# iglu-contest/gridworld

Measured on AMD Instinct MI355X. Metric: env-steps/sec (render=False, vector_state) at N parallel envs, 1/2/4/8 GPU, higher is better.
Workload: dtype f64

## Files before the change

__graft_entry__.py:

```python
import os
import sys

ROOT = os.path.dirname(os.path.abspath(__file__))
if ROOT not in sys.path:
    sys.path.insert(0, ROOT)


def build():
    from gridworld_amd import build as hip_build, codec as hip_codec, goal as hip_goal, query as hip_query, render as hip_render
    lib = hip_build.build(force=True)
    assert os.path.exists(lib)
    assert os.path.exists(hip_render.build(force=True))
    assert os.path.exists(hip_codec.build(force=True))
    assert os.path.exists(hip_query.build(force=True))
    assert os.path.exists(hip_goal.build(force=True))
    from oracle import oracle as O
    O.build(force=True)
    import gridworld_amd
    from gridworld_amd import _lib
    L = _lib.load()
    assert L.igw_version() == _lib.VERSION
    print('built', lib, 'and', O._LIB_PATH)


def smoke():
    import numpy as np
    import torch
    from gridworld_amd import VecGridWorld, workloads
    from oracle import oracle as O
    assert torch.cuda.is_available(), 'smoke() needs a GPU'

    def same(env, ob, n):
        torch.cuda.synchronize()
        assert np.array_equal(env.grid.cpu().numpy().reshape(n, -1), ob.grid)
        assert np.array_equal(env.agent_pos.cpu().numpy().view(np.uint32), ob.agentPos.view(np.uint32))
        assert np.array_equal(env.reward.cpu().numpy(), ob.reward) and np.array_equal(env.done.cpu().numpy(), ob.done)
        assert np.array_equal(env.inventory.cpu().numpy(), ob.inventory)
        assert np.array_equal(env.internals().view(np.uint64), ob.internals().view(np.uint64))

    n, T = 64, 60
    tg = workloads.rt20(n, seed=3).numpy()
    kw = dict(size_reward=False, max_steps=40)
    env = VecGridWorld(n, device='cuda:0', autoreset=True, **kw)
    env.set_tasks(tg)
# ... 42 lines not shown
```

gridworld_amd/_lib.py:

```python
import ctypes as C
import os

HERE = os.path.dirname(os.path.abspath(__file__))
LIB_PATH = os.path.join(HERE, 'libigw_hip.so')

GRID_STRIDE = 1104
CELLS = 1089
AGENT_BYTES = 64
AUX_BYTES = 16
OUT_BYTES = 64
TASK_META_BYTES = 128
OCC_WORDS = 48
TRAJ_BYTES = 64
HIST_ROW = 512
STAT_STRIPES = 64
STAT_CHANGED, STAT_RESETS, STAT_STEPS, STAT_RESCANS, STAT_BAD_POSE, STAT_BAD_ACTION, STAT_BAD_TASK = 0, 1, 2, 3, 4, 5, 6
VERSION = 5
LEVEL_INDEX_BYTES = 160
TASK_INDEX_BYTES = 9 * LEVEL_INDEX_BYTES
WALKING_DISCRETE, FLYING, WALKING_DICT = 0, 1, 2
RESET_KEEP_SIZE = 1
CAMERA_MAX = 1e6
AUTO_32_MAX, AUTO_16_MAX, AUTO_8_MAX = 1024, 4096, 24576

# ... 20 lines not shown


class Buffers(C.Structure):
    _fields_ = [(n, C.c_void_p) for n in ('grid', 'occ', 'hist', 'agent', 'aux', 'task_target', 'task_start',
                                          'task_start_occ', 'task_meta', 'task_index', 'out', 'stats')]


_lib = None


def load(build_if_missing=True):
    global _lib
    if _lib is not None:
        return _lib
    diag = os.environ.get('IGW_DIAG') == '1'
    path = os.path.join(HERE, 'libigw_hip_diag.so') if diag else LIB_PATH
    if os.environ.get('IGW_LIB'):
        path, build_if_missing = os.environ['IGW_LIB'], False
    if build_if_missing:
        from . import build as _build
        (_build.DIAG if diag else _build.STEP).build_for_load(IgwError)
    if not os.path.exists(path):
        raise IgwError(f'{os.path.basename(path)} not found; run `python -m gridworld_amd.build`')
    L = C.CDLL(path)
    vp, i32, i64, u64 = C.c_void_p, C.c_int32, C.c_int64, C.c_uint64
    L.igw_version.restype = C.c_int
    L.igw_last_error.restype = C.c_char_p
    L.igw_build_id.restype = C.c_char_p
    L.igw_device_count.restype = C.c_int
    L.igw_create.argtypes = [C.POINTER(Config), C.POINTER(vp)]
    L.igw_destroy.argtypes = [vp]
    L.igw_debug_set_stamps.argtypes = [vp, vp]
    L.igw_bind_buffers.argtypes = [vp, C.POINTER(Buffers)]
    L.igw_prepare_tasks.argtypes = [vp, i32, i32, vp, vp, vp, vp, vp, vp]
    L.igw_reset.argtypes = [vp, vp, i32, vp]
    L.igw_set_task_sampling.argtypes = [vp, i32, u64, i32]
    L.igw_set_random_tasks.argtypes = [vp, i32, u64, i32, i32, i32, i32, vp]
    L.igw_set_trajectory_log.argtypes = [vp, vp, vp, i32, i32]
    L.igw_step_walking.argtypes = [vp, vp, vp]
    L.igw_step_flying.argtypes = [vp, vp, vp, vp, vp, vp]
    L.igw_step_walking_dict.argtypes = [vp, vp, vp, vp]
    L.igw_rollout_walking.argtypes = [vp, i64, u64, i64, i64, vp]
    L.igw_rollout_walking_actions.argtypes = [vp, vp, i64, vp, vp, vp]
    L.igw_rollout_flying_actions.argtypes = [vp, vp, vp, vp, vp, i64, vp, vp, vp]
    L.igw_fill_actions_walking.argtypes = [vp, vp, i64, i64, u64, i64, vp]
    L.igw_task_eval.argtypes = [i32, i32, vp, vp, vp, vp, vp, vp, vp, vp]
    L.igw_debug_trig.argtypes = [i32, i64, vp, vp, vp, vp, vp, vp, vp]
    for name in EXPORTS:
        getattr(L, name)
        if name not in ('igw_last_error', 'igw_build_id'):
            getattr(L, name).restype = C.c_int
    _lib = L
    return L


def build_id():
    return load().igw_build_id().decode()


def check(code, what=''):
    if code != 0:
        msg = load().igw_last_error()
        raise IgwError(f'{what} failed ({code}): {msg.decode() if msg else ""}')
```

gridworld_amd/env.py:

```python
import ctypes as C
import warnings

import numpy as np
import torch

from . import _lib as L
from . import spaces
from .tasks import Task, Tasks
from .vec_env import VecGridWorld

_NO_TASK = ('Task is not initialized! Initialize task before working with the environment using .set_task '
            'method OR set tasks distribution using .set_task_generator method')
_TIS = (2, 4, 8, 12)


class AgentView:
    PAD = 0.25
    __slots__ = ('_env',)

    def __init__(self, env):
        self._env = env

    def _f64(self):
        return self._env._host['agent'][:48].view(np.float64)
# ... 137 lines not shown
            self._step_call = lambda: v.lib.igw_step_flying(v.ctx, p + 16, p + 8, p + 28, p + 32, self._stream_handle)
        elif v.walk_dict:
            self._step_call = lambda: v.lib.igw_step_walking_dict(v.ctx, p, p + 8, self._stream_handle)
        else:
            self._step_call = lambda: v.lib.igw_step_walking(v.ctx, p, self._stream_handle)
        self._read_back()
        self._frame = None
        if self.renderer_kind == 'hip':
            W, H = int(self.render_size[0]), int(self.render_size[1])
            self._frame = torch.zeros((1, H, W, 4), dtype=torch.uint8).pin_memory()

    def _launch_frame(self):
        from . import render as R
        v = self._vec
        R.render_into(v.agent_buf.data_ptr(), v.grid_buf.data_ptr(), v.occ_buf.data_ptr(), 1, v._atlas(),
                      self._frame.data_ptr(), self._frame.shape[2], self._frame.shape[1], 4, self._stream_handle)

    def _renders(self):
        return self.do_render and not self.fake and self._frame is not None

    def _device_step(self):
        rc = self._step_call()
        if rc:
            L.check(rc, 'igw_step (facade)')
        if self._renders():
            self._launch_frame()
        self._stream.synchronize()

    def _read_back(self):
        torch.cuda.current_stream(self._vec.device).synchronize()

    @property
    def unwrapped(self):
        return self

    @property
    def step_no(self):
        return int(self._host['agent'][60:62].view(np.uint16)[0])

    @property
    def grid(self):
        return self._host['grid'].reshape(9, 11, 11).astype(np.int32)

    def set_task(self, task):
        if self._task_generator is not None:
            warnings.warn('The .set_task method has no effect with an initialized tasks generator. '
                          'Drop it using .set_tasks_generator(None) after calling .set_task')
# ... 246 lines not shown
```

gridworld_amd/vec_env.py:

```python
import ctypes as C
import weakref

import numpy as np
import torch

from . import _lib as L
from . import codec as K
from . import goal as G
from . import query as Q
from . import render as R


def _as_rows(x, device, n=None):
    if x is None:
        return None
    t = torch.as_tensor(np.asarray(x) if not torch.is_tensor(x) else x)
    if t.dim() == 3:
        t = t.unsqueeze(0)
    t = t.reshape(t.shape[0], -1)
    if t.shape[1] == L.GRID_STRIDE:
        return t.to(device=device, dtype=torch.int8).contiguous()
    if t.shape[1] != L.CELLS:
        raise ValueError(f'grid rows must have 1089 cells, got {t.shape[1]}')
    out = torch.zeros((t.shape[0], L.GRID_STRIDE), dtype=torch.int8, device=device)
    out[:, :L.CELLS] = t.to(device=device, dtype=torch.int8)
    return out


def _invariant(x, n, device):
# ... 54 lines not shown
            self.dev = torch.zeros((2, self.n), dtype=torch.uint8, device=self.device)
            self.dev[0].fill_(int(root not in self.drawn))

    def captured(self, sl, restart):
        first, mask = self.dev[0, sl], self.dev[1, sl]
        if restart is None:
            mask.copy_(first)
        else:
            torch.bitwise_or(restart, first, out=mask)
        first.zero_()
        return mask


class _Rows:
    parent, lo, stream = None, 0, None

    def _root(self):
        return self if self.parent is None else self.parent

    def _open(self, cfg, stats_buf):
        root, sl = self._root(), slice(self.lo, self.lo + cfg.num_envs)
        self.cfg, self.num_envs, self.env_index_base, self.stats_buf = cfg, cfg.num_envs, cfg.env_index_base, stats_buf
        self.ctx = C.c_void_p()
        L.check(self.lib.igw_create(C.byref(cfg), C.byref(self.ctx)), 'igw_create')
        bound = [getattr(root, k)[sl] for k in _ROW_BUFFERS] + [getattr(root, k) for k in _TASK_BUFFERS] + \
            [root.out_buf[sl], stats_buf]
        L.check(self.lib.igw_bind_buffers(self.ctx, C.byref(L.Buffers(*[t.data_ptr() for t in bound]))),
                'igw_bind_buffers')
        self._sl = sl
        self._rows = (root.agent_buf[sl], root.grid_buf[sl], root.occ_buf[sl])

    def _follow_with(self, pov, mask, goal=None):
        self._pov, self._mask, self._goal = pov, mask, goal
        self.pov = pov.tensors.get('rgb') if pov else None
        self.pov_obs = pov.obs if pov else None
        self._obs = {'agentPos': self.agent_pos, 'inventory': self.inventory, 'compass': self.compass.unsqueeze(1),
                     'grid': self.grid}
        if pov is not None:
            pov.add_to(self._obs)
        if mask is not None:
            self._obs['action_mask'] = mask
        if goal is not None:
            self._obs.update(goal)
            if 'gain' in goal:
                self._goal_scratch()

    def __del__(self):
        ctx = getattr(self, 'ctx', None)
        if ctx:
            self.lib.igw_destroy(ctx)
            self.ctx = None

    def _stream(self):
        if self.stream is None:
            return C.c_void_p(torch._C._cuda_getCurrentRawStream(self._dev_index))
        return C.c_void_p(self.stream.cuda_stream)

    def _in_use(self, *tensors):
        if self.stream is not None:
            for t in tensors:
                if torch.is_tensor(t):
                    t.record_stream(self.stream)

    def _atlas(self):
        root = self._root()
        if root._render_atlas is None:
            root.set_render_atlas(None)
        return root._render_atlas

# ... 39 lines not shown
                                        torch.zeros((n, L.AGENT_BYTES), dtype=torch.uint8, device=dev),
                                        torch.zeros((n, Q.ACTIONS), dtype=torch.uint8, device=dev))
        return tmp

    def _ended(self):
        return self.done if self.autoreset else None

    def _draw(self, stream=None, restart=None, fill=False):
        pov = self._pov
        if stream is None:
            stream = self._stream()
            self._in_use(*pov.tensors.values(), pov.obs)
        if pov.obs is not None:
            _render_obs_rows(self, pov.spec, pov.obs, pov.tensors.get('rgb'), restart, fill, stream)
        elif pov.plain:
            _render_rows(self, pov.tensors['rgb'], 3, None, None, stream)
        else:
            _render_rows(self, pov.tensors, 3, None, tuple(pov.tensors), stream)

    def step_walking_ptr(self, actions_i32):
        if actions_i32.numel() != self.num_envs:
            raise _SPACES[L.WALKING_DISCRETE].mismatch('step_walking_ptr', self.num_envs, None, actions_i32)
        self._in_use(actions_i32)
        L.check(self.lib.igw_step_walking(self.ctx, actions_i32.data_ptr(), self._stream()), 'igw_step_walking')
        if self.parent is None:
            self._follow_mask()
            self._follow_goal()
        else:
            self._follow(self._ended())

    def action_mask(self, out=None, look=False, sample=None):
        self._in_use(*(out if isinstance(out, (tuple, list)) else (out,)))
        res = _mask_rows(self, out, look, sample, self._stream(), self.stream)
        self._in_use(*(res if isinstance(res, tuple) else (res,)))
        return res

    def goal(self, want=False, todo=True, gain=False, out=None):
        names = ('align', 'fit') + (('want',) if want else ()) + (('todo',) if todo else ()) + \
            (('gain', 'ends') if gain else ())
        self._in_use(*(out or {}).values())
        res = _goal_rows(self, names, out, self._stream(), self.stream)
        self._in_use(*res.values())
        return res

    def render_pov(self, out=None, channels=3, size=None, outputs=None, codec=None, quality=90):
        self._in_use(*(out.values() if isinstance(out, dict) else out if isinstance(out, (tuple, list)) else (out,)))

# ... 16 lines not shown
                 renderer=None, pov_outputs=('rgb',), pov_obs=None, pov_frame=True, action_mask=False, goal=False):
        if renderer not in (None, 'hip'):
            raise ValueError(f"unknown renderer {renderer!r}; the one renderer is 'hip'")
        pov_outputs = R.check_outputs(pov_outputs)
        if renderer is None and pov_outputs != ('rgb',):
            raise ValueError("pov_outputs needs renderer='hip'")
        if pov_obs is not None:
            if renderer is None:
                raise ValueError("pov_obs needs renderer='hip'")
            if pov_outputs != ('rgb',):
                raise ValueError("pov_obs goes with pov_outputs=('rgb',) only: the planes are not written in this layout")
            pov_obs = R.ObsSpec.of(pov_obs)
        elif not pov_frame:
            raise ValueError('pov_frame=False needs pov_obs (there would be nothing to draw)')
        if render and not fake and renderer is None:
            raise NotImplementedError("render=True needs renderer='hip' (the batched HIP ray caster of the "
                                      "first-person frame); or pass render=False")
        if not torch.cuda.is_available():
            raise L.IgwError('VecGridWorld needs a HIP device (no CPU fallback)')
        if action_space not in ('walking', 'flying'):
            raise ValueError(f'unknown action_space {action_space!r}')
        if action_mask and (action_space != 'walking' or not discretize):
            raise ValueError('action_mask=True needs the Discrete(18) walking action space')
        self.lib = L.load()
        self.device = torch.device(device)
        self.num_envs = int(num_envs)
        self.num_tasks = int(num_tasks or num_envs)
        self.flying = action_space == 'flying'
        self.walk_dict = action_space == 'walking' and not discretize
        mode = L.FLYING if self.flying else L.WALKING_DICT if self.walk_dict else L.WALKING_DISCRETE
        self._space = _SPACES[mode]
        self.max_steps = int(max_steps)
        self.autoreset = bool(autoreset)
        self.select_and_place = bool(select_and_place)
        N, T, dev = self.num_envs, self.num_tasks, self.device
        z = lambda shape, dt: torch.zeros(shape, dtype=dt, device=dev)
        rec = L.OUT_BYTES + L.AGENT_BYTES + L.AUX_BYTES
        self.host_records = bool(host_records)
        if self.host_records:
            self.host_view = torch.zeros((N * (rec + L.GRID_STRIDE),), dtype=torch.uint8).pin_memory()
        else:
            self.host_view = z((N * (rec + L.GRID_STRIDE),), torch.uint8)
        cut = lambda lo, width: self.host_view[N * lo:N * (lo + width)].view(N, width)
        self.out_buf = cut(0, L.OUT_BYTES)
        self.agent_buf = cut(L.OUT_BYTES, L.AGENT_BYTES)
        self.aux_buf = cut(L.OUT_BYTES + L.AGENT_BYTES, L.AUX_BYTES)
        self.grid_buf = cut(rec, L.GRID_STRIDE).view(torch.int8)
# ... 64 lines not shown
        dev = self.device
        tgt = _as_rows(targets, dev)
        T = tgt.shape[0]
        st = _as_rows(starts, dev)
        fg = _as_rows(full_grids, dev)
        inv = _invariant(invariant, T, dev)
        for name, g, hi in (('targets', tgt, 7), ('starts', st, 6), ('full_grids', fg, 7)):
            if g is not None and g.numel() and (int(g.min()) < 0 or int(g.max()) > hi):
                raise ValueError(f'{name}: block ids must be in 0..{hi}')
        if first < 0 or first + T > self.num_tasks:
            raise ValueError(f'task rows [{first}, {first + T}) do not fit the table of {self.num_tasks}')
        for name, g in (('starts', st), ('full_grids', fg)):
            if g is not None and g.shape[0] != T:
                raise ValueError(f'{name} has {g.shape[0]} rows, targets {T}')
        pose = None
        if init_pose is not None:
            pose_np = np.asarray(init_pose, dtype=np.float64).reshape(T, 5)
            ok = np.isfinite(pose_np).all() and (np.abs(pose_np[:, [0, 2]]) <= 10).all() and \
                (np.abs(pose_np[:, 1]) <= 64).all() and (np.abs(pose_np[:, 3:]) <= 1e6).all()
            if not ok:
                raise ValueError('init_pose must be finite with |x|, |z| <= 10, |y| <= 64 and |yaw|, |pitch| <= 1e6')
            pose = torch.as_tensor(pose_np, device=dev).contiguous()
        ptr = lambda t: None if t is None else C.c_void_p(t.data_ptr())
        L.check(self.lib.igw_prepare_tasks(self.ctx, first, T, ptr(tgt), ptr(st), ptr(fg), ptr(inv), ptr(pose),
                                           self._stream()), 'igw_prepare_tasks')
        if self.user_target is None:
            self.user_target = torch.zeros((self.num_tasks, L.GRID_STRIDE), dtype=torch.int8, device=dev)
        self.user_target[first:first + T] = tgt
        self._tasks_filled = max(self._tasks_filled, first + T)
        if env_task is not None:
            et = np.asarray(env_task.cpu() if torch.is_tensor(env_task) else env_task).reshape(-1)
            if et.shape[0] != self.num_envs or et.min() < 0 or et.max() >= self.num_tasks:
                raise ValueError(f'env_task needs {self.num_envs} indices into the task table [0, {self.num_tasks})')
            self.env_task.copy_(torch.as_tensor(et.astype(np.int32), device=dev))
        elif first == 0:
            if T == self.num_envs:
                self.env_task.copy_(torch.arange(self.num_envs, dtype=torch.int32, device=dev))
            elif T == 1:
                self.env_task.zero_()
        self._keep = (tgt, st, fg, inv, pose)
        self._have_tasks = True
        self._fill.raise_()

    def set_task_sampling(self, enabled=True, seed=0, n_tasks=None):
        n = int(n_tasks if n_tasks is not None else self._tasks_filled)
        if enabled and not 0 < n <= self.num_tasks:
            raise ValueError('set_task_sampling needs filled task rows: call set_tasks first')
        L.check(self.lib.igw_set_task_sampling(self.ctx, int(bool(enabled)), int(seed), n), 'igw_set_task_sampling')
        self._sampling = ('table', int(seed), n) if enabled else None
        self.config_epoch += 1
        for c in self._children:
            c._inherit_sampling()

    def set_random_tasks(self, enabled=True, seed=0, max_blocks=4, height_levels=1, max_dist=2, num_colors=1):
        kw = dict(max_blocks=int(max_blocks), height_levels=int(height_levels), max_dist=int(max_dist),
                  num_colors=int(num_colors))
        L.check(self.lib.igw_set_random_tasks(self.ctx, int(bool(enabled)), int(seed), kw['max_blocks'],
                                              kw['height_levels'], kw['max_dist'], kw['num_colors'], self._stream()),
                'igw_set_random_tasks')
        self._sampling = ('random', int(seed), kw) if enabled else None
        self.config_epoch += 1
        if enabled:
            self._have_tasks = True
            self._tasks_filled = max(self._tasks_filled, self.num_envs)
        for c in self._children:
            c._inherit_sampling()

    def targets(self):
        rows = self.task_target[self.env_task.long()]
        return rows[:, :L.CELLS].reshape(self.num_envs, 9, 11, 11)

    def enable_trajectory_log(self, n_envs=1, capacity=None):
        n_envs = int(n_envs)
        cap = int(capacity or self.max_steps)
        rec = torch.zeros((n_envs, 2, cap, L.TRAJ_BYTES), dtype=torch.uint8, device=self.device)
        heads = torch.zeros((n_envs, 2, 4), dtype=torch.int32, device=self.device)
        L.check(self.lib.igw_set_trajectory_log(self.ctx, rec.data_ptr(), heads.data_ptr(), n_envs, cap),
                'igw_set_trajectory_log')
        self._traj = (rec, heads, n_envs, cap)
        self.config_epoch += 1
        return rec, heads

    def disable_trajectory_log(self):
        L.check(self.lib.igw_set_trajectory_log(self.ctx, None, None, 0, 0), 'igw_set_trajectory_log')
        self._traj = None
        self.config_epoch += 1

    _STATE_KEYS = ('grid_buf', 'occ_buf', 'hist_buf', 'agent_buf', 'aux_buf', 'out_buf', 'task_target', 'task_start',
                   'task_start_occ', 'task_meta', 'task_index', 'stats_buf')

    def state_dict(self):
        d = {k: getattr(self, k).clone() for k in self._STATE_KEYS}
        d['abi_version'] = L.VERSION
        return d

    def load_state_dict(self, state):
        if state.get('abi_version') != L.VERSION:
            raise ValueError(f'state_dict is of ABI version {state.get("abi_version")!r}, this build is version {L.VERSION}')
        missing = [k for k in self._STATE_KEYS if k not in state]
        extra = [k for k in state if k not in self._STATE_KEYS and k != 'abi_version']
        if missing or extra:
            raise ValueError(f'state_dict keys do not match: missing {missing}, unexpected {extra}')
        for k in self._STATE_KEYS:
            if tuple(state[k].shape) != tuple(getattr(self, k).shape):
                raise ValueError(f'state_dict[{k!r}] has shape {tuple(state[k].shape)}, expected {tuple(getattr(self, k).shape)}')
        for k in self._STATE_KEYS:
            getattr(self, k).copy_(state[k])
        self._have_tasks = True
        self._follow(draw=False)

    def _need_tasks(self):
        if not self._have_tasks:
            raise ValueError('Task is not initialized! Initialize task before working with the environment '
                             'using .set_tasks')

    def dense(self):
        return {'agentPos': self.agent_pos.contiguous(), 'inventory': self.inventory.contiguous(),
                'compass': self.compass.contiguous(), 'reward': self.reward.contiguous(), 'done': self.done.contiguous()}

    def reset(self, mask=None, keep_size=False):
        self._need_tasks()
        m = None
        if mask is not None:
            m = torch.as_tensor(mask, device=self.device).to(torch.uint8).contiguous()
        L.check(self.lib.igw_reset(self.ctx, None if m is None else C.c_void_p(m.data_ptr()),
                                   L.RESET_KEEP_SIZE if keep_size else 0, self._stream()), 'igw_reset')
        self._mask_keep = m
        self._follow(None if m is None else m.reshape(-1), fill=m is None)
        return self.obs()

    @staticmethod
    def _check_camera(cam):
        if torch.is_tensor(cam):
            if cam.is_cuda:
                return
            c = cam.detach().numpy()
        else:
            c = np.asarray(cam)
        c = c.astype(np.float64, copy=False)
        if c.size and not (np.isfinite(c).all() and np.abs(c).max() <= L.CAMERA_MAX):
            raise ValueError(f'camera deltas must be finite with |value| <= {L.CAMERA_MAX:g} degrees')

    def step(self, actions):
        if not self._have_tasks:
            self._need_tasks()
        bufs = self._action_buffers(actions)
        sp = self._space
        rc = getattr(self.lib, sp.step)(self.ctx, *[b.data_ptr() for b in bufs],
                                         torch._C._cuda_getCurrentRawStream(self._dev_index))
        if rc:
            L.check(rc, sp.step)
        self._act_keep = bufs
        self._follow(self._ended())
        return self._obs.copy(), self.reward, self.done, {}

    def _action_buffers(self, actions, steps=None):
        sp, N, dev, bufs = self._space, self.num_envs, self.device, []
        for (key, dt, shape), count in zip(sp.buffers, sp.counts):
            if key is None:
                x = actions
            elif key == 'buttons' and steps is None and 'buttons' not in actions:
                x = torch.stack([torch.as_tensor(np.asarray(actions[k]), device=dev).to(dt).reshape(-1)
                                 for k in BUTTONS], dim=1)
            else:
                x = actions[key]
            if not (type(x) is torch.Tensor and x.dtype is dt and x.is_cuda and x.is_contiguous()):
                if steps == 'capture_steps':
                    raise ValueError(f'capture_steps: {key or "actions"} must be a contiguous {dt} device tensor '
                                     f'[T, {", ".join(map(str, (N, *shape)))}]')
                if key == 'camera':
                    self._check_camera(x)
                x = torch.as_tensor(x, device=dev).to(dt).contiguous()
            if steps is None:
                ok = x.numel() == N * count
# ... 22 lines not shown
            raise ValueError(f"what must be 'grid', 'target' or 'start', got {what!r}") from None
        kw.setdefault('size', self.render_size)
        if kw.get('atlas') is None:
            kw['atlas'] = self._atlas()
        return V.render_views(grids, poses, view_grid=rows, device=self.device, **kw)

    def capture_steps(self, actions, record=False, chains=1):
        self._need_tasks()
        return StepGraph(self, actions, record, chains)

    def _before_capture(self):
        if self._pov is not None:
            self._atlas()
            if self._pov.stacked:
                self._fill.on_device(self)

    def _replayed(self, chains):
        if self.pov_obs is not None:
            self._fill.lowered(self, *chains)
        return self._obs.copy(), self.reward, self.done, {}

    def rollout(self, T, seed, t0=0, env_offset=0):
        self._need_tasks()
        L.check(self.lib.igw_rollout_walking(self.ctx, int(T), int(seed), int(t0), int(env_offset),
                                             self._stream()), 'igw_rollout_walking')
        self._follow(draw=False)

    def rollout_actions(self, actions, return_rewards=False):
        self._need_tasks()
        N, dev, sp = self.num_envs, self.device, self._space
        if sp.rollout is None:
            raise L.IgwError('rollout_actions: Discrete(18) walking and flying only')
        if self._traj is not None:
            raise L.IgwError('rollout / rollout_actions do not write the episode log: disable_trajectory_log() first')
        bufs = self._action_buffers(actions, 'rollout_actions')
        T = int(bufs[0].shape[0])
        rw = dn = None
        if return_rewards:
            rw = torch.empty((T, N), dtype=torch.float32, device=dev)
            dn = torch.empty((T, N), dtype=torch.uint8, device=dev)
        rp, dp = (rw.data_ptr() if rw is not None else None), (dn.data_ptr() if dn is not None else None)
        L.check(getattr(self.lib, sp.rollout)(self.ctx, *[b.data_ptr() for b in bufs], T, rp, dp, self._stream()),
                sp.rollout)
        self._keep = bufs
        self._follow(draw=False)
        return (rw, dn) if return_rewards else None

    def fill_actions(self, n_steps, seed, t0=0, env_offset=0):
        a = torch.empty((n_steps, self.num_envs), dtype=torch.int32, device=self.device)
        L.check(self.lib.igw_fill_actions_walking(self.ctx, a.data_ptr(), int(n_steps), int(t0), int(seed),
                                                  int(env_offset), self._stream()), 'igw_fill_actions_walking')
        return a

    def split(self, parts, streams=None):
        if self.num_envs % parts:
            raise ValueError('num_envs must be divisible by parts')
        n = self.num_envs // parts
        streams = streams or [torch.cuda.Stream(device=self.device) for _ in range(parts)]
        cur = torch.cuda.current_stream(self.device)
        subs = []
        for k in range(parts):
            streams[k].wait_stream(cur)
            subs.append(SubBatch(self, k * n, n, streams[k]))
        self._children.extend(subs)
        return subs

    def _release_children(self, subs):
        for c in subs:
            if c in self._children:
                self.stats_buf += c.stats_buf
                self._children.remove(c)

    def stats_tensor(self):
        s = self.stats_buf.sum(0)
# ... 42 lines not shown
            raise L.IgwError('capture_steps(chains > 1) cannot be combined with the episode log or the RandomTasks generator')
        self.chains = chains
        self.config_epoch = env.config_epoch
        self._held = env._traj
        self.buffers = tuple(env._action_buffers(actions, 'capture_steps'))
        self.T = T = int(self.buffers[0].shape[0])
        if T < 1:
            raise ValueError('capture_steps: every action buffer needs the same number of steps T >= 1')
        self.outs = torch.zeros((T, N, L.OUT_BYTES), dtype=torch.uint8, device=dev) if record else None
        fn, row_bytes = getattr(env.lib, env._space.step), env._space.row_bytes
        self.graph = torch.cuda.CUDAGraph()
        cur = torch.cuda.current_stream(dev)
        self.subs = env.split(chains) if chains > 1 else None
        self.graphs = [self.graph] + [torch.cuda.CUDAGraph() for _ in range(chains - 1)]
        self.streams = [torch.cuda.Stream(device=dev) for _ in range(chains)]
        env._before_capture()
        for part, graph, st in zip(self.subs or [env], self.graphs, self.streams):
            st.wait_stream(cur)
            lo, n = part.lo, part.num_envs
            ptrs = [[b[t].data_ptr() + lo * rb for b, rb in zip(self.buffers, row_bytes)] for t in range(T)]
            with torch.cuda.graph(graph, stream=st, capture_error_mode='thread_local'):
                h = C.c_void_p(st.cuda_stream)
                for t in range(T):
                    L.check(fn(part.ctx, *ptrs[t], h), 'step (capture)')
                    if record:
                        self.outs[t, lo:lo + n].copy_(env.out_buf[lo:lo + n])
                    part._follow_captured(h, t == 0, t == T - 1)
            cur.wait_stream(st)
        if record:
            f = self.outs.view(torch.float32)
            self.rewards, self.dones = f[:, :, 12], self.outs[:, :, 52]

    def __del__(self):
        subs, env = getattr(self, 'subs', None), getattr(self, 'env', None)
        if subs and env is not None:
            try:
                env._release_children(subs)
            except Exception:
                pass

    def replay(self):
        env = self.env
        if env.config_epoch != self.config_epoch:
            raise L.IgwError('StepGraph is stale: set_task_sampling / set_random_tasks / enable_trajectory_log / '
                             'disable_trajectory_log was called after capture_steps (a captured launch carries those '
                             'settings by value); capture the steps again')
        if self.chains == 1:
# ... 15 lines not shown

    def __init__(self, parent, lo, n, stream):
        self.parent, self.lo, self.stream = parent, lo, stream
        for k in self._SHARED:
            setattr(self, k, getattr(parent, k))
        cfg = L.Config.from_buffer_copy(parent.cfg)
        cfg.num_envs = n
        cfg.env_index_base = parent.env_index_base + lo
        if cfg.lanes_per_env == 0:
            cfg.lanes_per_env = L.auto_lanes(parent.num_envs)
        self._open(cfg, torch.zeros_like(parent.stats_buf))
        sl = self._sl
        for k in self._VIEWS:
            setattr(self, k, getattr(parent, k)[sl])
        self._follow_with(parent._pov and parent._pov.rows(sl), None if parent._mask is None else parent._mask[sl],
                          None if parent._goal is None else {k: t[sl] for k, t in parent._goal.items()})
        if parent in parent._fill.drawn:
            parent._fill.lowered(self)
        self._inherit_sampling()

    def _inherit_sampling(self):
        sp = self.parent._sampling
        if sp is None:
            L.check(self.lib.igw_set_task_sampling(self.ctx, 0, 0, 0), 'igw_set_task_sampling')
            L.check(self.lib.igw_set_random_tasks(self.ctx, 0, 0, 1, 1, 1, 1, None), 'igw_set_random_tasks')
        elif sp[0] == 'table':
            L.check(self.lib.igw_set_task_sampling(self.ctx, 1, sp[1], sp[2]), 'igw_set_task_sampling')
        else:
            raise L.IgwError('the RandomTasks generator cannot be combined with sub-batches')

    def reset(self):
        L.check(self.lib.igw_reset(self.ctx, None, 0, self._stream()), 'igw_reset')
        self._follow(fill=True)
        return self.obs()

    def synchronize(self):
        self.stream.synchronize()

    def join(self):
        torch.cuda.current_stream(self.device).wait_stream(self.stream)


class _Pov:

    def __init__(self, tensors, spec=None, obs=None):
        self.tensors, self.spec, self.obs = tensors, spec, obs
        self.plain = tuple(tensors) == ('rgb',) and obs is None
        self.stacked = obs is not None and spec.stack > 1

    def rows(self, sl):
        return _Pov({k: t[sl] for k, t in self.tensors.items()}, self.spec, None if self.obs is None else self.obs[sl])

    def add_to(self, obs):
        for k, t in self.tensors.items():
            obs['pov' if k == 'rgb' else k] = t
# ... 73 lines not shown
```

Measured before the change: 6.483 billion.

## Add separate step library with specialized fast step kernel using DPP and staged resets

Builds a new step library that wraps the existing kernels and adds a specialized step kernel. It uses DPP row reductions and quad broadcasts to spread agent and aux records across each 4-lane group, and resolves changed-piece histograms in chunked passes with touched-bit tracking so only modified histogram rows are written back. It also prefetches reset rows into shared scratch while the world update runs. The environment now loads this library in place of the original, which adds a second build artifact and more specialized code paths that must stay bit-exact with the oracle.

```diff
diff --git a/__graft_entry__.py b/__graft_entry__.py
--- a/__graft_entry__.py
+++ b/__graft_entry__.py
@@ -7,9 +7,11 @@
 
 
 def build():
-    from gridworld_amd import build as hip_build, codec as hip_codec, goal as hip_goal, query as hip_query, render as hip_render
+    from gridworld_amd import build as hip_build, codec as hip_codec, goal as hip_goal, query as hip_query, render as hip_render, \
+        step_lib as hip_step
     lib = hip_build.build(force=True)
     assert os.path.exists(lib)
+    assert os.path.exists(hip_step.build(force=True))
     assert os.path.exists(hip_render.build(force=True))
     assert os.path.exists(hip_codec.build(force=True))
     assert os.path.exists(hip_query.build(force=True))
@@ -19,7 +21,7 @@
     import gridworld_amd
     from gridworld_amd import _lib
     L = _lib.load()
-    assert L.igw_version() == _lib.VERSION
+    assert L.igw_version() == _lib.VERSION == hip_step.load().igw_version()
     print('built', lib, 'and', O._LIB_PATH)
 
 
diff --git a/gridworld_amd/_lib.py b/gridworld_amd/_lib.py
--- a/gridworld_amd/_lib.py
+++ b/gridworld_amd/_lib.py
@@ -66,7 +66,11 @@
         (_build.DIAG if diag else _build.STEP).build_for_load(IgwError)
     if not os.path.exists(path):
         raise IgwError(f'{os.path.basename(path)} not found; run `python -m gridworld_amd.build`')
-    L = C.CDLL(path)
+    _lib = declare(C.CDLL(path))
+    return _lib
+
+
+def declare(L):
     vp, i32, i64, u64 = C.c_void_p, C.c_int32, C.c_int64, C.c_uint64
     L.igw_version.restype = C.c_int
     L.igw_last_error.restype = C.c_char_p
@@ -94,7 +98,6 @@
         getattr(L, name)
         if name not in ('igw_last_error', 'igw_build_id'):
             getattr(L, name).restype = C.c_int
-    _lib = L
     return L
 
 
diff --git a/gridworld_amd/csrc/step/igw_step.hip b/gridworld_amd/csrc/step/igw_step.hip
--- /dev/null
+++ b/gridworld_amd/csrc/step/igw_step.hip
@@ -0,0 +1,339 @@
+#include "../../../include/igw.h"
+
+#define igw_step_walking igw_step_walking_base
+#define igw_step_flying igw_step_flying_base
+#define igw_step_walking_dict igw_step_walking_dict_base
+#include "../igw_kernels.hip"
+#undef igw_step_walking
+#undef igw_step_flying
+#undef igw_step_walking_dict
+
+static_assert(IGW_SPLIT_BURST == 1 && IGW_EARLY_COUNTERS == 1 && IGW_UNTRACKED_DMA == 1, "step_kernel_fast is the shipped variant only");
+
+namespace igw {
+
+__device__ inline uint32_t row_or_all(uint32_t v) {
+    v |= (uint32_t)__builtin_amdgcn_update_dpp(0, (int)v, 0x121, 0xF, 0xF, false);
+    v |= (uint32_t)__builtin_amdgcn_update_dpp(0, (int)v, 0x122, 0xF, 0xF, false);
+    v |= (uint32_t)__builtin_amdgcn_update_dpp(0, (int)v, 0x124, 0xF, 0xF, false);
+    v |= (uint32_t)__builtin_amdgcn_update_dpp(0, (int)v, 0x128, 0xF, 0xF, false);
+    return v;
+}
+
+__device__ inline int resolve_changed_pieces(const Grp<4>& G, const KParams& p, WaveScratch<req_chunk<4>()>& ws, uint64_t mask,
+                                             int env, int task, const CellChange& ch, int start_val, uint32_t* spare) {
+    constexpr int GS = 4, R = req_chunk<GS>();
+    if (mask == 0) return 0;
+    const int lane = __lane_id();
+    const int E = __builtin_popcountll(mask);
+    uint64_t m = mask;
+    if (E > R) {
+#pragma unroll
+        for (int k = 0; k < R; k++) m &= m - 1;
+        const int l = __builtin_ctzll(m);
+        dma_change_rows<false>(p, spare, spare + HIST_ROW / 2, __builtin_amdgcn_readlane(env, l), __builtin_amdgcn_readlane(task, l),
+                               __builtin_amdgcn_readlane(ch.lvl, l));
+    }
+    const bool grp_changed = (mask >> (lane & ~(GS - 1))) & 1ull;
+    const int below = (int)__builtin_amdgcn_mbcnt_hi((uint32_t)(mask >> 32), __builtin_amdgcn_mbcnt_lo((uint32_t)mask, 0u));
+    const int rank = below - ((G.gl > 0 && grp_changed) ? 1 : 0);
+    if (grp_changed && G.gl == 0) {
+        const int a = old_colour(ch) - start_val, b = ch.new_val - start_val;
+        *reinterpret_cast<uint2*>(ws.chg[rank]) =
+            make_uint2((uint32_t)env, (uint32_t)ch.xz | (change_class(a) << 8) | (change_class(b) << 12));
+    }
+    const int slot = lane >> 4, sub = lane & 15, mi = sub >> 2, q = lane & 3;
+    int result = 0;
+    const auto pass = [&](int base, auto later) {
+        const int cnt = min(R, E - base);
+        wave_sync();
+        const bool my = slot < cnt;
+        const int sl = my ? slot : 0;
+        const uint2 ent = my ? *reinterpret_cast<const uint2*>(ws.chg[base + sl]) : make_uint2(0u, 0u);
+        uint32_t* hrow = ws.hist[sl];
+        const uint8_t* blk = reinterpret_cast<const uint8_t*>(ws.aux[sl]);
+        if constexpr (decltype(later)::value) {
+            if (base == R && sl == 0) {
+                hrow = spare;
+                blk = reinterpret_cast<const uint8_t*>(spare + HIST_ROW / 2);
+            }
+        }
+        const int gx = (int)(ent.y & 15u), gz = (int)((ent.y >> 4) & 15u);
+        const int ka = (int)((ent.y >> 8) & 15u), kb = (int)((ent.y >> 12) & 15u);
+        const int oa0 = blk[LVL_OFFS - 1 + ka], oa1 = blk[LVL_OFFS + ka], ob0 = blk[LVL_OFFS - 1 + kb], ob1 = blk[LVL_OFFS + kb];
+        const int na = (my && ka != 0) ? oa1 - oa0 : 0, n = na + ((my && kb != 0) ? ob1 - ob0 : 0);
+        const int bb = my ? (int)reinterpret_cast<const uint32_t*>(blk)[q] : 0;
+        const int xmin = (int)(int8_t)(bb & 0xff), dxlo = (int)(int8_t)((bb >> 8) & 0xff) - 10;
+        const int zmin = (int)(int8_t)((bb >> 16) & 0xff), dzlo = (int)(int8_t)((bb >> 24) & 0xff) - 10;
+        uint32_t touched_lo = 0, touched_hi = 0;
+        for (int i0 = 0;; i0 += 4) {
+            const int idx = i0 + mi;
+            const bool act = idx < n;
+            if (!__any(act)) break;
+            if (act) {
+                const bool dec = idx < na;
+                const int cell = blk[LVL_CELLS + (dec ? oa0 + idx : ob0 + (idx - na))];
+                const int tx = cell >> 4, tz = cell & 15;
+                const int bx = (q & 1) ? tz : tx, bz = (q & 1) ? tx : tz;
+                const int rx = q >= 2 ? 10 - bx : bx;
+                const int rz = (q == 1 || q == 2) ? 10 - bz : bz;
+                const int u = rx - gx - dxlo, v = rz - gz - dzlo;
+                if ((unsigned)u <= (unsigned)(xmin - dxlo) && (unsigned)v <= (unsigned)(zmin - dzlo)) {
+                    const int bin = q * 121 + __mul24(u, 11) + v;
+                    atomicAdd(&hrow[bin >> 1], (dec ? 0xffffffffu : 1u) << (16 * (bin & 1)));
+                    const uint32_t bit = 1u << ((bin >> 3) & 31);
+                    touched_lo |= bin < 256 ? bit : 0u;
+                    touched_hi |= bin < 256 ? 0u : bit;
+                }
+            }
+        }
+        wave_sync();
+        touched_lo = row_or_all(touched_lo);
+        touched_hi = row_or_all(touched_hi);
+        typedef unsigned short us2 __attribute__((ext_vector_type(2)));
+        us2 pm = {0, 0};
+        if (my) {
+            const uint4* row = reinterpret_cast<const uint4*>(hrow);
+            uint4* dst = reinterpret_cast<uint4*>(p.hist + (size_t)ent.x * HIST_ROW);
+#pragma unroll
+            for (int j = 0; j < 4; j++) {
+                const uint4 now = row[j * 16 + sub];
+                if (((j < 2 ? touched_lo : touched_hi) >> ((j & 1) * 16 + sub)) & 1u) dst[j * 16 + sub] = now;
+                pm = __builtin_elementwise_max(pm, __builtin_elementwise_max(
+                    __builtin_elementwise_max(__builtin_bit_cast(us2, now.x), __builtin_bit_cast(us2, now.y)),
+                    __builtin_elementwise_max(__builtin_bit_cast(us2, now.z), __builtin_bit_cast(us2, now.w))));
+            }
+        }
+        const int best = row_max_nonneg((int)max((uint32_t)pm.x, (uint32_t)pm.y));
+        const int mine = __builtin_amdgcn_ds_bpermute((((rank - base) & (R - 1)) * 16 + 15) * 4, best);
+        if (grp_changed && rank >= base && rank < base + R) result = mine;
+    };
+    pass(0, std::false_type{});
+    for (int base = R; base < E; base += R) {
+        const int cnt = min(R, E - base);
+#pragma unroll
+        for (int k = 0; k < R; k++) {
+            if (k < cnt) {
+                const int l = next_leader(m);
+                if (!(k == 0 && base == R))
+                    dma_change_inputs<R, false>(p, ws, k, __builtin_amdgcn_readlane(env, l), __builtin_amdgcn_readlane(task, l),
+                                                __builtin_amdgcn_readlane(ch.lvl, l));
+            }
+        }
+        asm volatile("s_waitcnt vmcnt(0)" ::: "memory");
+        pass(base, std::true_type{});
+    }
+    wave_sync();
+    return result;
+}
+
+template <int MODE, bool EXACT = false>
+__global__ __launch_bounds__(BLOCK, 4) void step_kernel_fast(const uint32_t* h_occ, const AgentRec* h_agent, const AuxRec* h_aux,
+                                                             const void* h_a0, const void* h_a1, const void* h_a2, const void* h_a3,
+                                                             KParams p, ActIn a) {
+    constexpr int GS = 4;
+    __shared__ BlockShared<GS> sh;
+    const Grp<GS> G;
+    TrigCtx trig;
+    trig.lut = trig_lut();
+    const int wave = __builtin_amdgcn_readfirstlane(threadIdx.x / WAVE);
+    const int slot = threadIdx.x / GS;
+    const int env = blockIdx.x * BlockShared<GS>::EPB + slot;
+    const int wave_env0 = blockIdx.x * BlockShared<GS>::EPB + wave * BlockShared<GS>::EPW;
+    static_assert(!EXACT || MODE == MODE_FLY, "EXACT is the flying kernel's variant");
+    const int n_envs = MODE != MODE_FLY ? (int)(uintptr_t)h_a3 : EXACT ? 0x7fffffff : p.n_envs;
+    const bool active = EXACT || env < n_envs;
+    uint32_t* occ_wave_s = sh.occ + wave * BlockShared<GS>::EPW * OCC_PITCH;
+    uint32_t* occ_s = sh.occ + slot * OCC_PITCH;
+    if (!EXACT && wave_env0 >= n_envs) return;
+    prio_at<true, 0>();
+    const int env_r = active ? env : n_envs - 1;
+    const bool writer = active && G.gl == 0;
+    OccStage<GS> occ_in = {};
+    AgentRec rec;
+    const uint4 rec_piece = reinterpret_cast<const uint4*>(h_agent + env_r)[G.gl & 3];
+    const uint32_t aux_w = reinterpret_cast<const uint32_t*>(h_aux + env_r)[G.gl & 3];
+    const ActIn ah = {(const int32_t*)h_a0, (const float*)h_a0, (const float*)h_a1, (const int32_t*)h_a2, (const int32_t*)h_a3,
+                      (const uint8_t*)h_a0};
+    RawAct ra = {};
+    if constexpr (MODE == MODE_FLY) load_fly_spread<GS>(ah, env_r, G.gl, ra);
+    else ra = load_action<MODE>(ah, env_r);
+    int8_t* grid_g = p.grid + (size_t)env_r * STRIDE;
+    occ_issue<GS>(h_occ, G, env_r, occ_in);
+    occ_commit_const<GS>(occ_wave_s);
+    uint4 rp = rec_piece;
+    uint32_t aw = aux_w;
+#if defined(__HIP_DEVICE_COMPILE__)
+    if constexpr (MODE == MODE_WALK)
+        asm volatile("" : "+v"(aw), "+v"(ra.action), "+v"(rp.x), "+v"(rp.y), "+v"(rp.z), "+v"(rp.w));
+    else if constexpr (MODE == MODE_FLY)
+        asm volatile("" : "+v"(aw), "+v"(ra.w1), "+v"(ra.w2), "+v"(rp.x), "+v"(rp.y), "+v"(rp.z), "+v"(rp.w));
+    else
+        asm volatile("" : "+v"(aw), "+v"(ra.buttons.x), "+v"(ra.buttons.y), "+v"(ra.f[3]), "+v"(ra.f[4]), "+v"(rp.x), "+v"(rp.y), "+v"(rp.z), "+v"(rp.w));
+#endif
+    {
+        uint32_t w[16];
+        const int px = (int)rp.x, py = (int)rp.y, pz = (int)rp.z, pw = (int)rp.w;
+        w[0] = (uint32_t)dpp_quad<QUAD_BCAST0>(px); w[1] = (uint32_t)dpp_quad<QUAD_BCAST0>(py);
+        w[2] = (uint32_t)dpp_quad<QUAD_BCAST0>(pz); w[3] = (uint32_t)dpp_quad<QUAD_BCAST0>(pw);
+        w[4] = (uint32_t)dpp_quad<QUAD_BCAST1>(px); w[5] = (uint32_t)dpp_quad<QUAD_BCAST1>(py);
+        w[6] = (uint32_t)dpp_quad<QUAD_BCAST1>(pz); w[7] = (uint32_t)dpp_quad<QUAD_BCAST1>(pw);
+        w[8] = (uint32_t)dpp_quad<QUAD_BCAST2>(px); w[9] = (uint32_t)dpp_quad<QUAD_BCAST2>(py);
+        w[10] = (uint32_t)dpp_quad<QUAD_BCAST2>(pz); w[11] = (uint32_t)dpp_quad<QUAD_BCAST2>(pw);
+        w[12] = (uint32_t)dpp_quad<QUAD_BCAST3>(px); w[13] = (uint32_t)dpp_quad<QUAD_BCAST3>(py);
+        w[14] = (uint32_t)dpp_quad<QUAD_BCAST3>(pz); w[15] = (uint32_t)dpp_quad<QUAD_BCAST3>(pw);
+        __builtin_memcpy(&rec, w, sizeof(rec));
+    }
+    const uint4 aux = make_uint4((uint32_t)dpp_quad<QUAD_BCAST0>((int)aw), (uint32_t)dpp_quad<QUAD_BCAST1>((int)aw),
+                                 (uint32_t)dpp_quad<QUAD_BCAST2>((int)aw), (uint32_t)dpp_quad<QUAD_BCAST3>((int)aw));
+    Env e;
+    env_unpack(e, rec, aux);
+    int task = (int)aux.z;
+    const int size_in = e.size;
+    const bool ends = p.autoreset && e.step_no + 1 >= p.max_steps;
+    const bool pre_ok = ends && !p.sample_tasks && !p.rt_enabled;
+    ResetMeta pre = reset_meta_any();
+    if (pre_ok) pre = load_reset_meta(p.task_meta + task);
+    const bool boost = __any(ends);
+    prio_at<true, 1>(boost);
+    e.step_no = min(e.step_no + 1, 65535);
+    CellChange ch;
+    Motion mv;
+    ActPre ap;
+    if (MODE == MODE_WALK) {
+        const WalkAct w = parse_walking_discrete(ra.action);
+        ap = world_act_pre<GS, MODE_WALK>(G, p, e, trig, w.s0, w.s1, w.dy, w.inventory, w.cam0, w.cam1, w.remove, w.add, mv);
+    } else if (MODE == MODE_WALK_DICT) {
+        const uint2 bw = ra.buttons;
+        const bool fwd = bw.x & 0xffu, back = bw.x & 0xff00u, left = bw.x & 0xff0000u, right = bw.x & 0xff000000u;
+        const bool jump = bw.y & 0xffu, attack = bw.y & 0xff00u, use = bw.y & 0xff0000u;
+        int hotbar = (int)(bw.y >> 24);
+        double c0 = (double)ra.f[3], c1 = (double)ra.f[4];
+        bool bad = false;
+        if (hotbar > 6) { hotbar = 0; bad = true; }
+        if (!camera_ok(c0)) { c0 = 0.0; bad = true; }
+        if (!camera_ok(c1)) { c1 = 0.0; bad = true; }
+        if (bad && writer) stat_add(p.stats, IGW_STAT_BAD_ACTION, 1);
+        const double s0 = (fwd ? -1.0 : 0.0) + (back ? 1.0 : 0.0), s1 = (left ? -1.0 : 0.0) + (right ? 1.0 : 0.0);
+        ap = world_act_pre<GS, MODE_WALK_DICT>(G, p, e, trig, s0, s1, jump ? 1.0 : 0.0, hotbar, c0, c1, attack, use, mv);
+    } else {
+        fly_fields(ra);
+        const int placement = ra.placement;
+        int inventory = ra.inventory;
+        double f[5] = {(double)ra.f[0], (double)ra.f[1], (double)ra.f[2], (double)ra.f[3], (double)ra.f[4]};
+        bool bad = false;
+        if ((unsigned)inventory > 6u) { inventory = 0; bad = true; }
+#pragma unroll
+        for (int i = 0; i < 5; i++) {
+            if (i < 3 ? !__builtin_isfinite(f[i]) : !camera_ok(f[i])) { f[i] = 0.0; bad = true; }
+        }
+        if (bad && writer) stat_add(p.stats, IGW_STAT_BAD_ACTION, 1);
+        ap = world_act_pre<GS, MODE_FLY>(G, p, e, trig, f[0], f[1], f[2], inventory, f[3], f[4], placement == 2, placement == 1, mv);
+    }
+    occ_commit_var<GS>(G, occ_in, occ_s);
+    wave_sync();
+    Hit h;
+    h.hit = false; h.have_prev = false;
+    h.bx = h.by = h.bz = h.px = h.py = h.pz = 0;
+    if (ap.want_sight) h = hit_test<GS, true>(G, occ_s, e.x, e.y, e.z, ap.vx, ap.vy, ap.vz, boost, sh.ws[wave].hist[0]);
+    ch = world_act_post<GS, false>(G, e, occ_s, grid_g, ap, h);
+    int start_val = 0, env_max_int = 0;
+    if (ch.idx >= 0) start_val = p.task_start[(size_t)task * STRIDE + ch.idx];
+    if (p.size_reward && e.step_no == 1) env_max_int = p.task_meta[task].env_max_int;
+    const bool changed = active && ch.idx >= 0;
+    const uint64_t chg_mask = prefetch_changes<GS, false>(G, p, sh.ws[wave], changed, env_r, task, ch);
+    int staged_leader = -1;
+    uint32_t staged_occ = aw;
+    if (boost) {
+        constexpr int R = req_chunk<GS>();
+        const uint64_t pm = __ballot(pre_ok && writer);
+        if (pm != 0 && __builtin_popcountll(chg_mask) < R) {
+            staged_leader = __builtin_ctzll(pm);
+            const int t_task = __builtin_amdgcn_readlane(task, staged_leader);
+            const int8_t* row0 = p.task_start + (size_t)t_task * STRIDE;
+            glds16u(row0, 16u * (uint32_t)G.lane, sh.ws[wave].hist[R - 1]);
+            if (G.lane < CHUNKS - WAVE) glds16u(row0 + 16 * WAVE, 16u * (uint32_t)G.lane, sh.ws[wave].aux[R - 1]);
+            if (G.lane < OCC_WORDS) staged_occ = gload(p.task_start_occ + (size_t)t_task * OCC_WORDS + G.lane);
+        }
+    }
+    const TailParams tp = tail_params(kernarg_again<STEP_KERNARG_HEAD>(p));
+    if (chg_mask != 0 && tp.stats != nullptr && G.lane == 0)
+        counter_add(tp.stats + (blockIdx.x & (IGW_STAT_STRIPES - 1)) * 8 + IGW_STAT_RESCANS, (unsigned long long)__builtin_popcountll(chg_mask));
+    prio_at<true, 3>(boost);
+    if (MODE == MODE_FLY) world_update<GS, MODE_FLY, true>(G, p, e, occ_s, mv, boost);
+    else world_update<GS, MODE_WALK, true>(G, p, e, occ_s, mv, boost);
+    finish_break(e, ch);
+    prio_at<true, 5>(boost);
+    if (chg_mask != 0 || staged_leader >= 0) asm volatile("s_waitcnt vmcnt(0)" ::: "memory");
+    asm volatile("" : "+v"(start_val), "+v"(env_max_int), "+v"(staged_occ));
+    asm volatile("" : "+v"(pre.a), "+v"(pre.b), "+v"(pre.c), "+v"(pre.d));
+    if (active)
+        st4(reinterpret_cast<uint4*>(p.agent + env) + G.gl, agent_piece(G.gl, e.x, e.y, e.z, e.yaw, e.pitch, e.vy, env_pack_piece3(e)));
+    const int size_new = e.prev_size + syn_size_delta(ch, start_val);
+    const bool need = size_new != e.prev_size;
+    if (chg_mask != 0) {
+        const uint64_t m_need = __ballot(need && active && G.gl == 0);
+        if (m_need != 0 && tp.stats != nullptr && G.lane == 0)
+            counter_add(tp.stats + (blockIdx.x & (IGW_STAT_STRIPES - 1)) * 8 + IGW_STAT_CHANGED, (unsigned long long)__builtin_popcountll(m_need));
+    }
+    const int hmax = resolve_changed_pieces(G, p, sh.ws[wave], chg_mask, env_r, task, ch, start_val, occ_wave_s);
+    int mi = e.max_int;
+    if (changed) {
+        if (need) {
+            mi = hmax;
+            e.dirty = 0;
+        } else {
+            e.dirty = 1;
+        }
+    }
+    prio_at<true, 6>(boost);
+    tail_step<GS, MODE, false>(G, kernarg_again<STEP_KERNARG_HEAD>(p), a, sh, wave, env, active, e, ch, task, env_max_int, size_new, mi, need, changed, grid_g, occ_s, boost, 0, pre, pre_ok, tp, size_in, staged_leader, staged_occ,
+                               EXACT ? BlockShared<GS>::EPB : min(BlockShared<GS>::EPB, n_envs - (int)blockIdx.x * BlockShared<GS>::EPB));
+}
+
+}
+
+static inline bool fast_ctx(const igw_ctx* ctx, int action_space) {
+    return ctx && ctx->bound && ctx->gs == 4 && !ctx->kp.rt_enabled && !ctx->kp.traj && ctx->cfg.action_space == action_space;
+}
+
+#define LAUNCH_FAST(KERNEL, A0, A1, A2, A3)                                                                               \
+    hipLaunchKernelGGL(KERNEL, dim3(env_blocks(ctx)), dim3(BLOCK), 0, (hipStream_t)stream, ctx->kp.occ, ctx->kp.agent,    \
+                       ctx->kp.aux, (const void*)(A0), (const void*)(A1), (const void*)(A2), (const void*)(A3), ctx->kp, a)
+
+extern "C" {
+
+int igw_step_walking(igw_ctx* ctx, const int32_t* actions, void* stream) {
+    if (!fast_ctx(ctx, IGW_WALKING_DISCRETE) || !actions) return igw_step_walking_base(ctx, actions, stream);
+    CHECK_CTX("igw_step_walking");
+    ActIn a = {actions, nullptr, nullptr, nullptr, nullptr, nullptr};
+    LAUNCH_FAST((step_kernel_fast<MODE_WALK>), actions, nullptr, nullptr, (uintptr_t)ctx->kp.n_envs);
+    HIP_TRY(hipGetLastError());
+    return IGW_OK;
+}
+
+int igw_step_flying(igw_ctx* ctx, const float* movement, const float* camera, const int32_t* inventory,
+                    const int32_t* placement, void* stream) {
+    if (!fast_ctx(ctx, IGW_FLYING) || !movement || !camera || !inventory || !placement)
+        return igw_step_flying_base(ctx, movement, camera, inventory, placement, stream);
+    CHECK_CTX("igw_step_flying");
+    ActIn a = {nullptr, movement, camera, inventory, placement, nullptr};
+    if (ctx->kp.n_envs % (BLOCK / 4) == 0)
+        LAUNCH_FAST((step_kernel_fast<MODE_FLY, true>), movement, camera, inventory, placement);
+    else
+        LAUNCH_FAST((step_kernel_fast<MODE_FLY>), movement, camera, inventory, placement);
+    HIP_TRY(hipGetLastError());
+    return IGW_OK;
+}
+
+int igw_step_walking_dict(igw_ctx* ctx, const uint8_t* buttons, const float* camera, void* stream) {
+    if (!fast_ctx(ctx, IGW_WALKING_DICT) || !buttons || !camera || ((uintptr_t)buttons & 7))
+        return igw_step_walking_dict_base(ctx, buttons, camera, stream);
+    CHECK_CTX("igw_step_walking_dict");
+    ActIn a = {nullptr, nullptr, camera, nullptr, nullptr, buttons};
+    LAUNCH_FAST((step_kernel_fast<MODE_WALK_DICT>), buttons, camera, nullptr, (uintptr_t)ctx->kp.n_envs);
+    HIP_TRY(hipGetLastError());
+    return IGW_OK;
+}
+
+}
diff --git a/gridworld_amd/env.py b/gridworld_amd/env.py
--- a/gridworld_amd/env.py
+++ b/gridworld_amd/env.py
@@ -183,7 +183,7 @@
     def _device_step(self):
         rc = self._step_call()
         if rc:
-            L.check(rc, 'igw_step (facade)')
+            self._vec._check(rc, 'igw_step (facade)')
         if self._renders():
             self._launch_frame()
         self._stream.synchronize()
diff --git a/gridworld_amd/step_lib.py b/gridworld_amd/step_lib.py
--- /dev/null
+++ b/gridworld_amd/step_lib.py
@@ -0,0 +1,55 @@
+import ctypes as C
+import os
+import sys
+
+from . import _lib
+from . import build as _build
+
+HERE = os.path.dirname(os.path.abspath(__file__))
+LIB = os.path.join(HERE, 'libigw_step.so')
+SOURCES = [os.path.join(_build.CSRC, 'step', 'igw_step.hip')]
+HEADERS = [os.path.join(_build.CSRC, f) for f in _build.SOURCES + _build.HEADERS]
+LIBRARY = _build.Library(LIB, SOURCES, HEADERS, 'igw-build-id:', 'IGW_BUILD_ID', deps=[__file__])
+source_hash, built_id, is_stale = LIBRARY.source_hash, LIBRARY.built_id, LIBRARY.is_stale
+EXPORTS = _lib.EXPORTS + ['igw_step_walking_base', 'igw_step_flying_base', 'igw_step_walking_dict_base']
+
+_loaded = None
+
+
+def use_base():
+    which = os.environ.get('IGW_STEP_LIB', '')
+    if which not in ('', 'base'):
+        raise _lib.IgwError(f"IGW_STEP_LIB={which!r}: the one value is 'base' (libigw_hip.so); unset = libigw_step.so")
+    return which == 'base' or bool(os.environ.get('IGW_LIB')) or os.environ.get('IGW_DIAG') == '1'
+
+
+def build(force=False, verbose=False):
+    return LIBRARY.build(force, verbose=verbose)
+
+
+def load(build_if_missing=True):
+    global _loaded
+    if use_base():
+        return _lib.load(build_if_missing)
+    if _loaded is not None:
+        return _loaded
+    if build_if_missing:
+        LIBRARY.build_for_load(_lib.IgwError)
+    if not os.path.exists(LIB):
+        raise _lib.IgwError('libigw_step.so not found; run `python -m gridworld_amd.step_lib`')
+    _loaded = _lib.declare(C.CDLL(LIB))
+    return _loaded
+
+
+def build_id():
+    return load().igw_build_id().decode()
+
+
+def check(code, what='', lib=None):
+    if code != 0:
+        msg = (lib or load()).igw_last_error()
+        raise _lib.IgwError(f'{what} failed ({code}): {msg.decode() if msg else ""}')
+
+
+if __name__ == '__main__':
+    print(build(force='--force' in sys.argv, verbose=True))
diff --git a/gridworld_amd/vec_env.py b/gridworld_amd/vec_env.py
--- a/gridworld_amd/vec_env.py
+++ b/gridworld_amd/vec_env.py
@@ -5,6 +5,7 @@
 import torch
 
 from . import _lib as L
+from . import step_lib as S
 from . import codec as K
 from . import goal as G
 from . import query as Q
@@ -105,11 +106,11 @@
         root, sl = self._root(), slice(self.lo, self.lo + cfg.num_envs)
         self.cfg, self.num_envs, self.env_index_base, self.stats_buf = cfg, cfg.num_envs, cfg.env_index_base, stats_buf
         self.ctx = C.c_void_p()
-        L.check(self.lib.igw_create(C.byref(cfg), C.byref(self.ctx)), 'igw_create')
+        self._check(self.lib.igw_create(C.byref(cfg), C.byref(self.ctx)), 'igw_create')
         bound = [getattr(root, k)[sl] for k in _ROW_BUFFERS] + [getattr(root, k) for k in _TASK_BUFFERS] + \
             [root.out_buf[sl], stats_buf]
-        L.check(self.lib.igw_bind_buffers(self.ctx, C.byref(L.Buffers(*[t.data_ptr() for t in bound]))),
-                'igw_bind_buffers')
+        self._check(self.lib.igw_bind_buffers(self.ctx, C.byref(L.Buffers(*[t.data_ptr() for t in bound]))),
+                    'igw_bind_buffers')
         self._sl = sl
         self._rows = (root.agent_buf[sl], root.grid_buf[sl], root.occ_buf[sl])
 
@@ -128,6 +129,9 @@
             if 'gain' in goal:
                 self._goal_scratch()
 
+    def _check(self, code, what):
+        S.check(code, what, self.lib)
+
     def __del__(self):
         ctx = getattr(self, 'ctx', None)
         if ctx:
@@ -213,7 +217,7 @@
         if actions_i32.numel() != self.num_envs:
             raise _SPACES[L.WALKING_DISCRETE].mismatch('step_walking_ptr', self.num_envs, None, actions_i32)
         self._in_use(actions_i32)
-        L.check(self.lib.igw_step_walking(self.ctx, actions_i32.data_ptr(), self._stream()), 'igw_step_walking')
+        self._check(self.lib.igw_step_walking(self.ctx, actions_i32.data_ptr(), self._stream()), 'igw_step_walking')
         if self.parent is None:
             self._follow_mask()
             self._follow_goal()
@@ -276,7 +280,7 @@
             raise ValueError(f'unknown action_space {action_space!r}')
         if action_mask and (action_space != 'walking' or not discretize):
             raise ValueError('action_mask=True needs the Discrete(18) walking action space')
-        self.lib = L.load()
+        self.lib = S.load()
         self.device = torch.device(device)
         self.num_envs = int(num_envs)
         self.num_tasks = int(num_tasks or num_envs)
@@ -387,8 +391,8 @@
                 raise ValueError('init_pose must be finite with |x|, |z| <= 10, |y| <= 64 and |yaw|, |pitch| <= 1e6')
             pose = torch.as_tensor(pose_np, device=dev).contiguous()
         ptr = lambda t: None if t is None else C.c_void_p(t.data_ptr())
-        L.check(self.lib.igw_prepare_tasks(self.ctx, first, T, ptr(tgt), ptr(st), ptr(fg), ptr(inv), ptr(pose),
-                                           self._stream()), 'igw_prepare_tasks')
+        self._check(self.lib.igw_prepare_tasks(self.ctx, first, T, ptr(tgt), ptr(st), ptr(fg), ptr(inv), ptr(pose),
+                                               self._stream()), 'igw_prepare_tasks')
         if self.user_target is None:
             self.user_target = torch.zeros((self.num_tasks, L.GRID_STRIDE), dtype=torch.int8, device=dev)
         self.user_target[first:first + T] = tgt
@@ -411,7 +415,7 @@
         n = int(n_tasks if n_tasks is not None else self._tasks_filled)
         if enabled and not 0 < n <= self.num_tasks:
             raise ValueError('set_task_sampling needs filled task rows: call set_tasks first')
-        L.check(self.lib.igw_set_task_sampling(self.ctx, int(bool(enabled)), int(seed), n), 'igw_set_task_sampling')
+        self._check(self.lib.igw_set_task_sampling(self.ctx, int(bool(enabled)), int(seed), n), 'igw_set_task_sampling')
         self._sampling = ('table', int(seed), n) if enabled else None
         self.config_epoch += 1
         for c in self._children:
@@ -420,9 +424,9 @@
     def set_random_tasks(self, enabled=True, seed=0, max_blocks=4, height_levels=1, max_dist=2, num_colors=1):
         kw = dict(max_blocks=int(max_blocks), height_levels=int(height_levels), max_dist=int(max_dist),
                   num_colors=int(num_colors))
-        L.check(self.lib.igw_set_random_tasks(self.ctx, int(bool(enabled)), int(seed), kw['max_blocks'],
-                                              kw['height_levels'], kw['max_dist'], kw['num_colors'], self._stream()),
-                'igw_set_random_tasks')
+        self._check(self.lib.igw_set_random_tasks(self.ctx, int(bool(enabled)), int(seed), kw['max_blocks'],
+                                                  kw['height_levels'], kw['max_dist'], kw['num_colors'], self._stream()),
+                    'igw_set_random_tasks')
         self._sampling = ('random', int(seed), kw) if enabled else None
         self.config_epoch += 1
         if enabled:
@@ -440,14 +444,14 @@
         cap = int(capacity or self.max_steps)
         rec = torch.zeros((n_envs, 2, cap, L.TRAJ_BYTES), dtype=torch.uint8, device=self.device)
         heads = torch.zeros((n_envs, 2, 4), dtype=torch.int32, device=self.device)
-        L.check(self.lib.igw_set_trajectory_log(self.ctx, rec.data_ptr(), heads.data_ptr(), n_envs, cap),
-                'igw_set_trajectory_log')
+        self._check(self.lib.igw_set_trajectory_log(self.ctx, rec.data_ptr(), heads.data_ptr(), n_envs, cap),
+                    'igw_set_trajectory_log')
         self._traj = (rec, heads, n_envs, cap)
         self.config_epoch += 1
         return rec, heads
 
     def disable_trajectory_log(self):
-        L.check(self.lib.igw_set_trajectory_log(self.ctx, None, None, 0, 0), 'igw_set_trajectory_log')
+        self._check(self.lib.igw_set_trajectory_log(self.ctx, None, None, 0, 0), 'igw_set_trajectory_log')
         self._traj = None
         self.config_epoch += 1
 
@@ -488,8 +492,8 @@
         m = None
         if mask is not None:
             m = torch.as_tensor(mask, device=self.device).to(torch.uint8).contiguous()
-        L.check(self.lib.igw_reset(self.ctx, None if m is None else C.c_void_p(m.data_ptr()),
-                                   L.RESET_KEEP_SIZE if keep_size else 0, self._stream()), 'igw_reset')
+        self._check(self.lib.igw_reset(self.ctx, None if m is None else C.c_void_p(m.data_ptr()),
+                                       L.RESET_KEEP_SIZE if keep_size else 0, self._stream()), 'igw_reset')
         self._mask_keep = m
         self._follow(None if m is None else m.reshape(-1), fill=m is None)
         return self.obs()
@@ -514,7 +518,7 @@
         rc = getattr(self.lib, sp.step)(self.ctx, *[b.data_ptr() for b in bufs],
                                          torch._C._cuda_getCurrentRawStream(self._dev_index))
         if rc:
-            L.check(rc, sp.step)
+            self._check(rc, sp.step)
         self._act_keep = bufs
         self._follow(self._ended())
         return self._obs.copy(), self.reward, self.done, {}
@@ -583,8 +587,8 @@
 
     def rollout(self, T, seed, t0=0, env_offset=0):
         self._need_tasks()
-        L.check(self.lib.igw_rollout_walking(self.ctx, int(T), int(seed), int(t0), int(env_offset),
-                                             self._stream()), 'igw_rollout_walking')
+        self._check(self.lib.igw_rollout_walking(self.ctx, int(T), int(seed), int(t0), int(env_offset),
+                                                 self._stream()), 'igw_rollout_walking')
         self._follow(draw=False)
 
     def rollout_actions(self, actions, return_rewards=False):
@@ -601,16 +605,16 @@
             rw = torch.empty((T, N), dtype=torch.float32, device=dev)
             dn = torch.empty((T, N), dtype=torch.uint8, device=dev)
         rp, dp = (rw.data_ptr() if rw is not None else None), (dn.data_ptr() if dn is not None else None)
-        L.check(getattr(self.lib, sp.rollout)(self.ctx, *[b.data_ptr() for b in bufs], T, rp, dp, self._stream()),
-                sp.rollout)
+        self._check(getattr(self.lib, sp.rollout)(self.ctx, *[b.data_ptr() for b in bufs], T, rp, dp, self._stream()),
+                    sp.rollout)
         self._keep = bufs
         self._follow(draw=False)
         return (rw, dn) if return_rewards else None
 
     def fill_actions(self, n_steps, seed, t0=0, env_offset=0):
         a = torch.empty((n_steps, self.num_envs), dtype=torch.int32, device=self.device)
-        L.check(self.lib.igw_fill_actions_walking(self.ctx, a.data_ptr(), int(n_steps), int(t0), int(seed),
-                                                  int(env_offset), self._stream()), 'igw_fill_actions_walking')
+        self._check(self.lib.igw_fill_actions_walking(self.ctx, a.data_ptr(), int(n_steps), int(t0), int(seed),
+                                                      int(env_offset), self._stream()), 'igw_fill_actions_walking')
         return a
 
     def split(self, parts, streams=None):
@@ -699,7 +703,7 @@
             with torch.cuda.graph(graph, stream=st, capture_error_mode='thread_local'):
                 h = C.c_void_p(st.cuda_stream)
                 for t in range(T):
-                    L.check(fn(part.ctx, *ptrs[t], h), 'step (capture)')
+                    part._check(fn(part.ctx, *ptrs[t], h), 'step (capture)')
                     if record:
                         self.outs[t, lo:lo + n].copy_(env.out_buf[lo:lo + n])
                     part._follow_captured(h, t == 0, t == T - 1)
@@ -761,15 +765,15 @@
     def _inherit_sampling(self):
         sp = self.parent._sampling
         if sp is None:
-            L.check(self.lib.igw_set_task_sampling(self.ctx, 0, 0, 0), 'igw_set_task_sampling')
-            L.check(self.lib.igw_set_random_tasks(self.ctx, 0, 0, 1, 1, 1, 1, None), 'igw_set_random_tasks')
+            self._check(self.lib.igw_set_task_sampling(self.ctx, 0, 0, 0), 'igw_set_task_sampling')
+            self._check(self.lib.igw_set_random_tasks(self.ctx, 0, 0, 1, 1, 1, 1, None), 'igw_set_random_tasks')
         elif sp[0] == 'table':
-            L.check(self.lib.igw_set_task_sampling(self.ctx, 1, sp[1], sp[2]), 'igw_set_task_sampling')
+            self._check(self.lib.igw_set_task_sampling(self.ctx, 1, sp[1], sp[2]), 'igw_set_task_sampling')
         else:
             raise L.IgwError('the RandomTasks generator cannot be combined with sub-batches')
 
     def reset(self):
-        L.check(self.lib.igw_reset(self.ctx, None, 0, self._stream()), 'igw_reset')
+        self._check(self.lib.igw_reset(self.ctx, None, 0, self._stream()), 'igw_reset')
         self._follow(fill=True)
         return self.obs()
 
```

Result: no change. 6.474 billion (-0.1%).
